# iiscleap/ICL-speech-text-LLM

Measured on AMD Instinct MI355X. Metric: ICL utterances/sec (whole node), SALMONN+Llama2-7B 5-shot VOXCELEB, higher is better.
Workload: dtype bf16

## Files before the change

### icl-speech-text-llm_amd/csrc/norm.hip

```cpp
#include "common.h"

namespace {

constexpr int NT = 256;
constexpr int MAXN = 8192;

#ifndef ICL_NORM_NT
#define ICL_NORM_NT 0
#endif
__device__ __forceinline__ f32x4 load4(const void* base, int64_t off, int dtype) {
  if (dtype == ICL_F32) return ICL_NORM_NT ? __builtin_nontemporal_load((const f32x4*)((const float*)base + off)) : *(const f32x4*)((const float*)base + off);
  const u32x2 raw = *(const u32x2*)((const unsigned short*)base + off);
  return f32x4{__uint_as_float(raw[0] << 16), __uint_as_float(raw[0] & 0xffff0000u),
               __uint_as_float(raw[1] << 16), __uint_as_float(raw[1] & 0xffff0000u)};
}
__device__ __forceinline__ void store4(void* base, int64_t off, int dtype, f32x4 v) {
  if (dtype == ICL_F32) {
    *(f32x4*)((float*)base + off) = v;
  } else {
    u32x2 pk = {pack_bf16x2(v[0], v[1]), pack_bf16x2(v[2], v[3])};
    *(u32x2*)((unsigned short*)base + off) = pk;
  }
}

template <bool RMS, int MAXV, bool HOIST>
__global__ __launch_bounds__(NT) void norm_kernel(const void* x, int64_t ldx, const void* res,
                                                   float alpha, const float* gamma,
                                                   const float* beta, void* y, int64_t ldy,
                                                   void* y2, int64_t ldy2, int M, int N, float eps,
                                                   int in_dtype, int out_dtype) {
  const int lane = threadIdx.x & 63;
  const int64_t m = (int64_t)blockIdx.x * 4 + (threadIdx.x >> 6);
  if (m >= M) return;
  const int nvec = N >> 2;
  f32x4 v[MAXV];
  float s = 0.f;
#pragma unroll
  for (int i = 0; i < MAXV; ++i) {
    const int c = lane + i * 64;
    v[i] = f32x4{0.f, 0.f, 0.f, 0.f};
    if (c < nvec) {
      v[i] = load4(x, m * ldx + c * 4, in_dtype);
      if (res) {
        const f32x4 r = load4(res, m * ldx + c * 4, in_dtype);
        v[i] = v[i] + alpha * r;
      }
      s += RMS ? (v[i][0] * v[i][0] + v[i][1] * v[i][1] + v[i][2] * v[i][2] + v[i][3] * v[i][3])
               : (v[i][0] + v[i][1] + v[i][2] + v[i][3]);
    }
  }
  f32x4 gv[HOIST ? MAXV : 1], bv[(HOIST && !RMS) ? MAXV : 1];
  if (HOIST) {
#pragma unroll
    for (int i = 0; i < MAXV; ++i) {
      const int c = lane + i * 64;
      if (c < nvec) {
        gv[i] = *(const f32x4*)(gamma + c * 4);
        if (!RMS) bv[i] = *(const f32x4*)(beta + c * 4);
      }
    }
  }
  float mean = 0.f, rstd;
  if (RMS) {
    rstd = rsqrtf(wave_reduce_sum(s) / (float)N + eps);
  } else {
    mean = wave_reduce_sum(s) / (float)N;
    float q = 0.f;
#pragma unroll
    for (int i = 0; i < MAXV; ++i) {
      const int c = lane + i * 64;
      if (c < nvec) {
#pragma unroll
        for (int r = 0; r < 4; ++r) {
          const float d = v[i][r] - mean;
          q += d * d;
        }
      }
    }
    rstd = rsqrtf(wave_reduce_sum(q) / (float)N + eps);
  }
#pragma unroll
  for (int i = 0; i < MAXV; ++i) {
    const int c = lane + i * 64;
    if (c < nvec) {
      const f32x4 g = HOIST ? gv[i] : *(const f32x4*)(gamma + c * 4);
      f32x4 o;
      if (RMS) {
        o = v[i] * rstd * g;
      } else {
        const f32x4 b = HOIST ? bv[i] : *(const f32x4*)(beta + c * 4);
        o = (v[i] - mean) * rstd * g + b;
      }
      store4(y, m * ldy + c * 4, out_dtype, o);
      if (y2) store4(y2, m * ldy2 + c * 4, ICL_BF16, o);
    }
  }
}

__device__ __forceinline__ void load8(const void* base, int64_t off, int dtype, float (&v)[8]) {
  if (dtype == ICL_F32) {
    const f32x4 a = ICL_NORM_NT ? __builtin_nontemporal_load((const f32x4*)((const float*)base + off)) : *(const f32x4*)((const float*)base + off);
    const f32x4 b = ICL_NORM_NT ? __builtin_nontemporal_load((const f32x4*)((const float*)base + off + 4)) : *(const f32x4*)((const float*)base + off + 4);
#pragma unroll
    for (int r = 0; r < 4; ++r) { v[r] = a[r]; v[4 + r] = b[r]; }
  } else {
    const u32x4 raw = *(const u32x4*)((const unsigned short*)base + off);
#pragma unroll
    for (int r = 0; r < 4; ++r) { v[2 * r] = __uint_as_float(raw[r] << 16); v[2 * r + 1] = __uint_as_float(raw[r] & 0xffff0000u); }
  }
}
__device__ __forceinline__ void store8(void* base, int64_t off, int dtype, const float (&v)[8]) {
  if (dtype == ICL_F32) {
    *(f32x4*)((float*)base + off) = f32x4{v[0], v[1], v[2], v[3]};
    *(f32x4*)((float*)base + off + 4) = f32x4{v[4], v[5], v[6], v[7]};
  } else {
    u32x4 pk = {pack_bf16x2(v[0], v[1]), pack_bf16x2(v[2], v[3]), pack_bf16x2(v[4], v[5]), pack_bf16x2(v[6], v[7])};
    *(u32x4*)((unsigned short*)base + off) = pk;
  }
}

template <bool RMS, int MAXC>
__global__ __launch_bounds__(NT) void norm8_kernel(const void* x, int64_t ldx, const void* res, float alpha,
                                                    const float* gamma, const float* beta, void* y, int64_t ldy,
                                                    void* y2, int64_t ldy2, int M, int N, float eps, int in_dtype,
                                                    int out_dtype) {
  const int lane = threadIdx.x & 63;
  const int wave = blockIdx.x * 4 + (threadIdx.x >> 6), n_waves = gridDim.x * 4;
  const int nch = N >> 3;
  float cur[MAXC][8], nxt[MAXC][8];
  auto load_row = [&](int64_t m, float (&dst)[MAXC][8]) {
#pragma unroll
    for (int i = 0; i < MAXC; ++i) {
      const int c = lane + i * 64;
      if (c < nch) {
        load8(x, m * ldx + c * 8, in_dtype, dst[i]);
        if (res) {
          float r[8];
          load8(res, m * ldx + c * 8, in_dtype, r);
#pragma unroll
          for (int e = 0; e < 8; ++e) dst[i][e] += alpha * r[e];
        }
      }
    }
  };
  int64_t m = wave;
  if (m < M) load_row(m, cur);
  for (; m < M; m += n_waves) {
    const bool more = m + n_waves < M;
    if (more) load_row(m + n_waves, nxt);
    float s = 0.f;
#pragma unroll
    for (int i = 0; i < MAXC; ++i)
      if (lane + i * 64 < nch) {
#pragma unroll
        for (int e = 0; e < 8; ++e) s += RMS ? cur[i][e] * cur[i][e] : cur[i][e];
      }
    float mean = 0.f, rstd;
    if (RMS) {
      rstd = rsqrtf(wave_reduce_sum(s) / (float)N + eps);
    } else {
      mean = wave_reduce_sum(s) / (float)N;
      float q = 0.f;
#pragma unroll
      for (int i = 0; i < MAXC; ++i)
        if (lane + i * 64 < nch) {
#pragma unroll
          for (int e = 0; e < 8; ++e) {
            const float d = cur[i][e] - mean;
            q += d * d;
          }
        }
      rstd = rsqrtf(wave_reduce_sum(q) / (float)N + eps);
    }
#pragma unroll
    for (int i = 0; i < MAXC; ++i) {
      const int c = lane + i * 64;
      if (c < nch) {
        float g[8], o[8];
        load8(gamma, c * 8, ICL_F32, g);
        if (RMS) {
#pragma unroll
          for (int e = 0; e < 8; ++e) o[e] = cur[i][e] * rstd * g[e];
        } else {
          float b[8];
          load8(beta, c * 8, ICL_F32, b);
#pragma unroll
          for (int e = 0; e < 8; ++e) o[e] = (cur[i][e] - mean) * rstd * g[e] + b[e];
        }
        store8(y, m * ldy + c * 8, out_dtype, o);
        if (y2) store8(y2, m * ldy2 + c * 8, ICL_BF16, o);
      }
    }
    if (more) {
#pragma unroll
      for (int i = 0; i < MAXC; ++i)
#pragma unroll
        for (int e = 0; e < 8; ++e) cur[i][e] = nxt[i][e];
    }
  }
}

template <bool RMS>
void launch_norm(hipStream_t st, const void* x, int64_t ldx, const void* res, float alpha, const float* gamma,
                 const float* beta, void* y, int64_t ldy, void* y2, int64_t ldy2, int M, int N, float eps,
                 int in_dtype, int out_dtype) {
  const dim3 block(NT);
  const bool a32 = ((uintptr_t)x % (in_dtype == ICL_F32 ? 16 : 16)) == 0 && (!res || ((uintptr_t)res % 16) == 0) &&
                   ((uintptr_t)y % 16) == 0 && (!y2 || ((uintptr_t)y2 % 16) == 0) && ((uintptr_t)gamma % 16) == 0 &&
                   (RMS || ((uintptr_t)beta % 16) == 0);
  const int pl8 = ((N >> 3) + 63) / 64;
#ifndef ICL_NORM8_ALL
#define ICL_NORM8_ALL 0
#endif
  if (N % 8 == 0 && ldx % 8 == 0 && ldy % 8 == 0 && !res && !y2 && a32 && N <= 5120 && (ICL_NORM8_ALL || pl8 == 3 || pl8 > 8)) {
    static int n_cu = 0;
    if (n_cu <= 0) {
      n_cu = icl_device_cu_count();
      if (n_cu <= 0) n_cu = 256;
    }
    const int per_lane8 = ((N >> 3) + 63) / 64;
    const dim3 pgrid(min((M + 3) / 4, n_cu * (per_lane8 <= 3 ? 8 : 4)));
#define ICL_NORM8_CASE(C)                                                                                              \
  hipLaunchKernelGGL((norm8_kernel<RMS, C>), pgrid, block, 0, st, x, ldx, res, alpha, gamma, beta, y, ldy, y2, ldy2, M, N, \
                     eps, in_dtype, out_dtype)
    if (per_lane8 <= 2) ICL_NORM8_CASE(2);
    else if (per_lane8 <= 3) ICL_NORM8_CASE(3);
    else if (per_lane8 <= 8) ICL_NORM8_CASE(8);
    else ICL_NORM8_CASE(10);
#undef ICL_NORM8_CASE
    return;
  }
  const dim3 grid((M + 3) / 4);
  const int per_lane = ((N >> 2) + 63) / 64;
  const bool few_rows = M <= 2048;
#define ICL_NORM_CASE(V)                                                                                                  \
  do {                                                                                                                    \
    constexpr bool CAN = V * (RMS ? 2 : 3) * 4 <= 200;                                \
    if (CAN && few_rows)                                                                                                  \
      hipLaunchKernelGGL((norm_kernel<RMS, V, CAN>), grid, block, 0, st, x, ldx, res, alpha, gamma, beta, y, ldy, y2, ldy2, M, \
                         N, eps, in_dtype, out_dtype);                                                                    \
    else                                                                                                                  \
      hipLaunchKernelGGL((norm_kernel<RMS, V, false>), grid, block, 0, st, x, ldx, res, alpha, gamma, beta, y, ldy, y2, ldy2, \
                         M, N, eps, in_dtype, out_dtype);                                                                 \
  } while (0)
  if (per_lane <= 3) ICL_NORM_CASE(3);
  else if (per_lane <= 5) ICL_NORM_CASE(5);
  else if (per_lane <= 8) ICL_NORM_CASE(8);
  else if (per_lane <= 16) ICL_NORM_CASE(16);
  else if (per_lane <= 20) ICL_NORM_CASE(20);
  else ICL_NORM_CASE(32);
#undef ICL_NORM_CASE
}

int check_common(const char* name, const void* x, int64_t ldx, const float* gamma, void* y,
                 int64_t ldy, int M, int N, int in_dtype, int out_dtype) {
  ICL_CHECK_ARG(x && gamma && y, "%s: NULL pointer", name);
  ICL_CHECK_ARG(M > 0 && N > 0, "%s: M,N must be > 0", name);
  ICL_CHECK_ARG(N % 4 == 0 && N <= MAXN, "%s: N=%d must be a multiple of 4 and <= %d", name, N,
                MAXN);
  ICL_CHECK_ARG(ldx % 4 == 0 && ldy % 4 == 0 && ldx >= N && ldy >= N, "%s: bad leading dimensions", name);
  ICL_CHECK_ARG((in_dtype == ICL_F32 || in_dtype == ICL_BF16) && (out_dtype == ICL_F32 || out_dtype == ICL_BF16),
                "%s: bad dtype", name);
  ICL_CHECK_ARG(((uintptr_t)x % (in_dtype == ICL_F32 ? 16 : 8)) == 0 &&
                    ((uintptr_t)y % (out_dtype == ICL_F32 ? 16 : 8)) == 0 && ((uintptr_t)gamma % 16) == 0,
                "%s: misaligned pointer", name);
  return ICL_OK;
}

}

extern "C" int icl_layernorm(const void* x, int64_t ldx, const void* res, float alpha,
                             const float* gamma, const float* beta, void* y, int64_t ldy, void* y2,
                             int64_t ldy2, int32_t M, int32_t N, float eps, int32_t in_dtype,
                             int32_t out_dtype, void* stream) {
  int rc = check_common("icl_layernorm", x, ldx, gamma, y, ldy, M, N, in_dtype, out_dtype);
  if (rc) return rc;
  ICL_CHECK_ARG(beta && ((uintptr_t)beta % 16) == 0, "icl_layernorm: beta NULL or misaligned");
  if (y2) ICL_CHECK_ARG(ldy2 % 4 == 0 && ldy2 >= N && ((uintptr_t)y2 % 8) == 0, "icl_layernorm: bad y2");
  if (res) ICL_CHECK_ARG(((uintptr_t)res % (in_dtype == ICL_F32 ? 16 : 8)) == 0, "icl_layernorm: res misaligned");
  launch_norm<false>((hipStream_t)stream, x, ldx, res, alpha, gamma, beta, y, ldy, y2, ldy2, M, N, eps, in_dtype, out_dtype);
  ICL_CHECK_LAUNCH("icl_layernorm");
  return ICL_OK;
}

extern "C" int icl_rmsnorm(const void* x, int64_t ldx, const float* gamma, void* y, int64_t ldy,
                           int32_t M, int32_t N, float eps, int32_t in_dtype, int32_t out_dtype,
                           void* stream) {
  int rc = check_common("icl_rmsnorm", x, ldx, gamma, y, ldy, M, N, in_dtype, out_dtype);
  if (rc) return rc;
  launch_norm<true>((hipStream_t)stream, x, ldx, nullptr, 0.f, gamma, nullptr, y, ldy, nullptr, 0, M, N, eps, in_dtype, out_dtype);
  ICL_CHECK_LAUNCH("icl_rmsnorm");
  return ICL_OK;
}
```

Baseline: 145.2.

## Stage norm gamma/beta in LDS for large-row cases with persistent grid

Result: no change. 145.9 (median of 6 runs) (+0.5%).

```diff
diff --git a/icl-speech-text-llm_amd/csrc/norm.hip b/icl-speech-text-llm_amd/csrc/norm.hip
--- a/icl-speech-text-llm_amd/csrc/norm.hip
+++ b/icl-speech-text-llm_amd/csrc/norm.hip
@@ -5,11 +5,8 @@
 constexpr int NT = 256;
 constexpr int MAXN = 8192;
 
-#ifndef ICL_NORM_NT
-#define ICL_NORM_NT 0
-#endif
 __device__ __forceinline__ f32x4 load4(const void* base, int64_t off, int dtype) {
-  if (dtype == ICL_F32) return ICL_NORM_NT ? __builtin_nontemporal_load((const f32x4*)((const float*)base + off)) : *(const f32x4*)((const float*)base + off);
+  if (dtype == ICL_F32) return *(const f32x4*)((const float*)base + off);
   const u32x2 raw = *(const u32x2*)((const unsigned short*)base + off);
   return f32x4{__uint_as_float(raw[0] << 16), __uint_as_float(raw[0] & 0xffff0000u),
                __uint_as_float(raw[1] << 16), __uint_as_float(raw[1] & 0xffff0000u)};
@@ -97,10 +94,91 @@
   }
 }
 
+template <bool RMS, int MAXV>
+__global__ __launch_bounds__(NT) void norm_lds_kernel(const void* x, int64_t ldx, const void* res, float alpha,
+                                                       const float* gamma, const float* beta, void* y, int64_t ldy,
+                                                       void* y2, int64_t ldy2, int M, int N, float eps, int in_dtype,
+                                                       int out_dtype) {
+  __shared__ f32x4 sg[MAXV * 64];
+  __shared__ f32x4 sb[RMS ? 1 : MAXV * 64];
+  const int lane = threadIdx.x & 63;
+  const int nvec = N >> 2;
+  const int64_t n_waves = (int64_t)gridDim.x * 4;
+  f32x4 v[MAXV];
+  auto load_row = [&](int64_t r, f32x4 (&dst)[MAXV]) {
+#pragma unroll
+    for (int i = 0; i < MAXV; ++i) {
+      const int c = lane + i * 64;
+      if (c < nvec) {
+        dst[i] = load4(x, r * ldx + c * 4, in_dtype);
+        if (res) {
+          const f32x4 rr = load4(res, r * ldx + c * 4, in_dtype);
+          dst[i] = dst[i] + alpha * rr;
+        }
+      }
+    }
+  };
+  int64_t m = (int64_t)blockIdx.x * 4 + (threadIdx.x >> 6);
+  if (m < M) load_row(m, v);
+  for (int c = threadIdx.x; c < nvec; c += NT) {
+    sg[c] = *(const f32x4*)(gamma + c * 4);
+    if (!RMS) sb[c] = *(const f32x4*)(beta + c * 4);
+  }
+  __syncthreads();
+  for (; m < M; m += n_waves) {
+    float s = 0.f;
+#pragma unroll
+    for (int i = 0; i < MAXV; ++i)
+      if (lane + i * 64 < nvec) {
+        if (RMS) {
+#pragma clang fp contract(off)
+          const f32x4 sq = v[i] * v[i];
+          s += sq[0] + sq[1] + sq[2] + sq[3];
+        } else {
+          s += v[i][0] + v[i][1] + v[i][2] + v[i][3];
+        }
+      }
+    float mean = 0.f, rstd;
+    if (RMS) {
+      rstd = rsqrtf(wave_reduce_sum(s) / (float)N + eps);
+    } else {
+      mean = wave_reduce_sum(s) / (float)N;
+      float q = 0.f;
+#pragma unroll
+      for (int i = 0; i < MAXV; ++i)
+        if (lane + i * 64 < nvec) {
+#pragma unroll
+          for (int r = 0; r < 4; ++r) {
+            const float d = v[i][r] - mean;
+            q += d * d;
+          }
+        }
+      rstd = rsqrtf(wave_reduce_sum(q) / (float)N + eps);
+    }
+#pragma unroll
+    for (int i = 0; i < MAXV; ++i) {
+      const int c = lane + i * 64;
+      if (c < nvec) {
+        const f32x4 g = sg[c];
+        f32x4 o;
+        if (RMS) {
+          o = v[i] * rstd * g;
+        } else {
+          const f32x4 b = sb[c];
+          o = (v[i] - mean) * rstd * g + b;
+        }
+        store4(y, m * ldy + c * 4, out_dtype, o);
+        if (y2) store4(y2, m * ldy2 + c * 4, ICL_BF16, o);
+      }
+    }
+    if (m + n_waves < M) load_row(m + n_waves, v);
+  }
+}
+
 __device__ __forceinline__ void load8(const void* base, int64_t off, int dtype, float (&v)[8]) {
   if (dtype == ICL_F32) {
-    const f32x4 a = ICL_NORM_NT ? __builtin_nontemporal_load((const f32x4*)((const float*)base + off)) : *(const f32x4*)((const float*)base + off);
-    const f32x4 b = ICL_NORM_NT ? __builtin_nontemporal_load((const f32x4*)((const float*)base + off + 4)) : *(const f32x4*)((const float*)base + off + 4);
+    const f32x4 a = *(const f32x4*)((const float*)base + off);
+    const f32x4 b = *(const f32x4*)((const float*)base + off + 4);
 #pragma unroll
     for (int r = 0; r < 4; ++r) { v[r] = a[r]; v[4 + r] = b[r]; }
   } else {
@@ -119,7 +197,7 @@
   }
 }
 
-template <bool RMS, int MAXC>
+template <bool RMS, int MAXC, bool LDS>
 __global__ __launch_bounds__(NT) void norm8_kernel(const void* x, int64_t ldx, const void* res, float alpha,
                                                     const float* gamma, const float* beta, void* y, int64_t ldy,
                                                     void* y2, int64_t ldy2, int M, int N, float eps, int in_dtype,
@@ -127,6 +205,8 @@
   const int lane = threadIdx.x & 63;
   const int wave = blockIdx.x * 4 + (threadIdx.x >> 6), n_waves = gridDim.x * 4;
   const int nch = N >> 3;
+  __shared__ f32x4 sg[LDS ? MAXC * 128 : 1];
+  __shared__ f32x4 sb[(LDS && !RMS) ? MAXC * 128 : 1];
   float cur[MAXC][8], nxt[MAXC][8];
   auto load_row = [&](int64_t m, float (&dst)[MAXC][8]) {
 #pragma unroll
@@ -145,6 +225,22 @@
   };
   int64_t m = wave;
   if (m < M) load_row(m, cur);
+  if (LDS) {
+    for (int c = threadIdx.x; c < 2 * nch; c += NT) {
+      sg[(c & 1) * nch + (c >> 1)] = *(const f32x4*)(gamma + c * 4);
+      if (!RMS) sb[(c & 1) * nch + (c >> 1)] = *(const f32x4*)(beta + c * 4);
+    }
+    __syncthreads();
+  }
+  auto load_param = [&](const f32x4* sp, const float* gp, int c, float (&p)[8]) {
+    if (LDS) {
+      const f32x4 a = sp[c], b = sp[nch + c];
+#pragma unroll
+      for (int r = 0; r < 4; ++r) { p[r] = a[r]; p[4 + r] = b[r]; }
+    } else {
+      load8(gp, c * 8, ICL_F32, p);
+    }
+  };
   for (; m < M; m += n_waves) {
     const bool more = m + n_waves < M;
     if (more) load_row(m + n_waves, nxt);
@@ -177,13 +273,13 @@
       const int c = lane + i * 64;
       if (c < nch) {
         float g[8], o[8];
-        load8(gamma, c * 8, ICL_F32, g);
+        load_param(sg, gamma, c, g);
         if (RMS) {
 #pragma unroll
           for (int e = 0; e < 8; ++e) o[e] = cur[i][e] * rstd * g[e];
         } else {
           float b[8];
-          load8(beta, c * 8, ICL_F32, b);
+          load_param(sb, beta, c, b);
 #pragma unroll
           for (int e = 0; e < 8; ++e) o[e] = (cur[i][e] - mean) * rstd * g[e] + b[e];
         }
@@ -198,6 +294,24 @@
         for (int e = 0; e < 8; ++e) cur[i][e] = nxt[i][e];
     }
   }
+}
+
+int cu_count() {
+  static int n_cu = 0;
+  if (n_cu <= 0) {
+    n_cu = icl_device_cu_count();
+    if (n_cu <= 0) n_cu = 256;
+  }
+  return n_cu;
+}
+
+template <bool RMS, int V>
+int lds_blocks_per_cu() {
+  static int n = 0;
+  if (n <= 0) {
+    if (hipOccupancyMaxActiveBlocksPerMultiprocessor(&n, norm_lds_kernel<RMS, V>, NT, 0) != hipSuccess || n <= 0) n = 2;
+  }
+  return n;
 }
 
 template <bool RMS>
@@ -205,43 +319,43 @@
                  const float* beta, void* y, int64_t ldy, void* y2, int64_t ldy2, int M, int N, float eps,
                  int in_dtype, int out_dtype) {
   const dim3 block(NT);
-  const bool a32 = ((uintptr_t)x % (in_dtype == ICL_F32 ? 16 : 16)) == 0 && (!res || ((uintptr_t)res % 16) == 0) &&
+  const bool few_rows = M <= 2048;
+  const bool a32 = ((uintptr_t)x % 16) == 0 && (!res || ((uintptr_t)res % 16) == 0) &&
                    ((uintptr_t)y % 16) == 0 && (!y2 || ((uintptr_t)y2 % 16) == 0) && ((uintptr_t)gamma % 16) == 0 &&
                    (RMS || ((uintptr_t)beta % 16) == 0);
   const int pl8 = ((N >> 3) + 63) / 64;
-#ifndef ICL_NORM8_ALL
-#define ICL_NORM8_ALL 0
-#endif
-  if (N % 8 == 0 && ldx % 8 == 0 && ldy % 8 == 0 && !res && !y2 && a32 && N <= 5120 && (ICL_NORM8_ALL || pl8 == 3 || pl8 > 8)) {
-    static int n_cu = 0;
-    if (n_cu <= 0) {
-      n_cu = icl_device_cu_count();
-      if (n_cu <= 0) n_cu = 256;
-    }
-    const int per_lane8 = ((N >> 3) + 63) / 64;
-    const dim3 pgrid(min((M + 3) / 4, n_cu * (per_lane8 <= 3 ? 8 : 4)));
-#define ICL_NORM8_CASE(C)                                                                                              \
-  hipLaunchKernelGGL((norm8_kernel<RMS, C>), pgrid, block, 0, st, x, ldx, res, alpha, gamma, beta, y, ldy, y2, ldy2, M, N, \
-                     eps, in_dtype, out_dtype)
-    if (per_lane8 <= 2) ICL_NORM8_CASE(2);
-    else if (per_lane8 <= 3) ICL_NORM8_CASE(3);
-    else if (per_lane8 <= 8) ICL_NORM8_CASE(8);
+  if (N % 8 == 0 && ldx % 8 == 0 && ldy % 8 == 0 && !res && !y2 && a32 && N <= 5120 && (pl8 == 3 || pl8 > 8)) {
+    const dim3 pgrid(min((M + 3) / 4, cu_count() * (pl8 <= 3 ? 8 : 4)));
+#define ICL_NORM8_CASE(C)                                                                                                 \
+  do {                                                                                                                    \
+    if (few_rows)                                                                                                         \
+      hipLaunchKernelGGL((norm8_kernel<RMS, C, false>), pgrid, block, 0, st, x, ldx, res, alpha, gamma, beta, y, ldy, y2, ldy2, \
+                         M, N, eps, in_dtype, out_dtype);                                                                 \
+    else                                                                                                                  \
+      hipLaunchKernelGGL((norm8_kernel<RMS, C, true>), pgrid, block, 0, st, x, ldx, res, alpha, gamma, beta, y, ldy, y2, ldy2, \
+                         M, N, eps, in_dtype, out_dtype);                                                                 \
+  } while (0)
+    if (pl8 <= 3) ICL_NORM8_CASE(3);
     else ICL_NORM8_CASE(10);
 #undef ICL_NORM8_CASE
     return;
   }
   const dim3 grid((M + 3) / 4);
   const int per_lane = ((N >> 2) + 63) / 64;
-  const bool few_rows = M <= 2048;
 #define ICL_NORM_CASE(V)                                                                                                  \
   do {                                                                                                                    \
     constexpr bool CAN = V * (RMS ? 2 : 3) * 4 <= 200;                                \
     if (CAN && few_rows)                                                                                                  \
       hipLaunchKernelGGL((norm_kernel<RMS, V, CAN>), grid, block, 0, st, x, ldx, res, alpha, gamma, beta, y, ldy, y2, ldy2, M, \
                          N, eps, in_dtype, out_dtype);                                                                    \
-    else                                                                                                                  \
+    else if (few_rows || V < 5)                                                                                           \
       hipLaunchKernelGGL((norm_kernel<RMS, V, false>), grid, block, 0, st, x, ldx, res, alpha, gamma, beta, y, ldy, y2, ldy2, \
                          M, N, eps, in_dtype, out_dtype);                                                                 \
+    else {                                                                                                                \
+      const dim3 lgrid(V >= 16 && (res || y2) ? min((M + 3) / 4, cu_count() * lds_blocks_per_cu<RMS, V>()) : (M + 3) / 4); \
+      hipLaunchKernelGGL((norm_lds_kernel<RMS, V>), lgrid, block, 0, st, x, ldx, res, alpha, gamma, beta, y, ldy, y2, ldy2, \
+                         M, N, eps, in_dtype, out_dtype);                                                                 \
+    }                                                                                                                     \
   } while (0)
   if (per_lane <= 3) ICL_NORM_CASE(3);
   else if (per_lane <= 5) ICL_NORM_CASE(5);
```
